# westlake-repl/IDvs.MoRec

Hardware: AMD Instinct MI355X
Metric: user-sequences/sec end-to-end train step, SASRec+BERT-base (higher is better)
Workload: dtype fp16

## Files before the change

### idvs/morec_amd/_lib.py

```python
from __future__ import annotations

import ctypes as C
import os

import torch

_HERE = os.path.dirname(os.path.abspath(__file__))
LIB_PATH = os.environ.get("MOREC_HIP_LIB") or os.path.join(_HERE, "libmorec_hip.so")

F32, BF16, F16 = 0, 1, 2
ACT_NONE, ACT_GELU, ACT_RELU = 0, 1, 2
DACT_MUL = 3


class MorecError(RuntimeError):
    pass


class GemmDesc(C.Structure):
    _fields_ = [("M", C.c_int), ("N", C.c_int), ("K", C.c_int), ("lda", C.c_int), ("ldb", C.c_int), ("ldc", C.c_int),
                ("in_dtype", C.c_int), ("out_dtype", C.c_int), ("act", C.c_int), ("dact", C.c_int),
                ("accumulate", C.c_int), ("split_k", C.c_int), ("alpha", C.c_float), ("aux_deriv", C.c_int)]


# ... 59 lines not shown
    "morec_colsum": (C.c_int, [_P, _P, C.c_int, C.c_int, C.c_int, C.c_int, _P]),
    "morec_layernorm_fwd": (C.c_int, [_P, _P, _P, _P, C.c_int, _P, _P, C.c_float, _P, _P, _P, _P, C.c_int, C.c_int,
                                      C.c_int, C.c_float, C.c_uint64, C.c_float, C.c_uint64, _P, C.c_int, _P]),
    "morec_layernorm_bwd": (C.c_int, [_P, _P, _P, _P, _P, _P, _P, _P, _P, _P, _P, C.c_int, C.c_int, C.c_int, C.c_float,
                                      C.c_uint64, C.c_float, C.c_uint64, _P, _P, C.c_int, _P]),
    "morec_layernorm_fwd_res32": (C.c_int, [_P, _P, _P, _P, C.c_int, _P, _P, C.c_float, _P, _P, _P, _P, _P, C.c_int, C.c_int,
                                            C.c_int, C.c_float, C.c_uint64, C.c_float, C.c_uint64, _P]),
    "morec_layernorm_fwd_res32_pre": (C.c_int, [_P, _P, _P, _P, _P, _P, _P, _P, _P, C.c_float, _P, _P, _P, _P, C.c_int, C.c_int, C.c_int,
                                                C.c_float, C.c_uint64, _P]),
    "morec_layernorm_bwd_res32": (C.c_int, [_P, _P, _P, _P, _P, _P, _P, _P, _P, _P, _P, C.c_int, C.c_int, C.c_int, C.c_float,
                                            C.c_uint64, C.c_float, C.c_uint64, _P]),
    "morec_pos_grad": (C.c_int, [_P, _P, C.c_int, C.c_int, C.c_int, C.c_int, _P]),
    "morec_attn_fwd": (C.c_int, [C.POINTER(AttnDesc), _P, _P, _P, _P]),
    "morec_attn_bwd": (C.c_int, [C.POINTER(AttnDesc), _P, _P, _P, _P, _P]),
    "morec_attn_bwd_dbias": (C.c_int, [C.POINTER(AttnDesc), _P, _P, _P, _P, C.c_int, _P, _P, C.c_size_t, _P]),
    "morec_bert_embed_fwd": (C.c_int, [_P, _P, _P, _P, _P, _P, C.c_float, _P, _P, _P, _P, C.c_int, C.c_int, C.c_int,
                                       C.c_int, C.c_float, C.c_uint64, _P]),
    "morec_bert_embed_bwd": (C.c_int, [_P, _P, _P, _P, _P, C.c_int, C.c_int, C.c_int, C.c_int, C.c_int, _P, _P]),
    "morec_gather_rows": (C.c_int, [_P, _P, _P, C.c_int, C.c_int, C.c_int, _P]),
    "morec_scatter_add_rows": (C.c_int, [_P, _P, _P, C.c_int, C.c_int, C.c_int, C.c_int, _P]),
    "morec_indexed_rows_copy": (C.c_int, [_P, _P, _P, _P, C.c_int, C.c_int, C.c_int, _P]),
    "morec_strided_rows_copy": (C.c_int, [_P, _P, C.c_int, C.c_int, C.c_int, C.c_int, C.c_int, _P]),
    "morec_inbatch_ce_workspace_bytes": (C.c_size_t, [C.POINTER(CeDesc)]),
    "morec_inbatch_ce_fwd": (C.c_int, [C.POINTER(CeDesc), _P, _P, _P, _P, _P, _P, _P, _P, _P, _P, _P, _P]),
    "morec_inbatch_ce_bwd": (C.c_int, [C.POINTER(CeDesc), _P, _P, _P, _P, _P, _P, _P, _P, _P, C.c_float, _P, _P, _P,
                                       _P]),
    "morec_bce_fwd": (C.c_int, [_P, _P, _P, _P, _P, C.c_int, C.c_int, C.c_int, C.c_int, _P]),
    "morec_bce_bwd": (C.c_int, [_P, _P, _P, _P, _P, _P, _P, C.c_int, C.c_int, C.c_int, C.c_int, _P]),
    "morec_adamw": (C.c_int, [_P, _P, _P, _P, _P, C.c_size_t, C.c_float, C.c_float, C.c_float, C.c_float, C.c_float,
                              C.c_int, C.c_float, _P]),
# ... 60 lines not shown
```

### idvs/morec_amd/csrc/attention.hip

```cpp
#include <stdio.h>
#include <stdlib.h>
#include "common.hpp"

namespace {
template <int TB>
struct Tile {
    static constexpr int TP = 8 * TB;
    static constexpr int PP = TP + 4;
};

struct AttnArgs {
    const void* qkv;
    const float* key_keep;
    void* ctx;
    void* dqkv;
    int n_seq, T, n_heads, dh;
    int causal;
    float scale, mask_value;
    DropRng drop;
    const int32_t* cu;
    int total_rows;
};

template <typename T, int DC, int TB>
// ... 610 lines not shown
int check_desc(const morec_attn_desc* d) {
    if (!d) return MOREC_E_ARG;
    if (d->n_seq <= 0 || d->T <= 0 || d->n_heads <= 0 || d->dh <= 0) return MOREC_E_ARG;
    if (d->T > T_MAX) return MOREC_E_UNSUPPORTED;
    if (d->dh % 8) return MOREC_E_ALIGN;
    if (d->p_drop < 0.f || d->p_drop >= 1.f) return MOREC_E_ARG;
    if (d->total_rows < 0 || d->spare_rows_max < 0 || (d->spare_rows_max > 0 && (!d->cu_seqlens || d->total_rows <= 0))) return MOREC_E_ARG;
    return MOREC_OK;
}
}
int attn_spare_blocks(const morec_attn_desc* d) { return (d->cu_seqlens && d->total_rows > 0) ? (d->spare_rows_max + 15) / 16 : 0; }

int morec_attn_mfma_launch(const morec_attn_desc* d, const void* qkv, const float* key_keep, void* ctx_or_dctx,
                           void* dqkv, bool backward, hipStream_t s, float* csum = nullptr);
int colsum_f32_launch(const float* in, float* out, int rows, int N, hipStream_t s);
int morec_attn_f32mfma_launch(const morec_attn_desc* d, const void* qkv, const float* key_keep, void* ctx_or_dctx, void* dqkv, bool backward,
                              hipStream_t s);

static void warn_valu_fallback(const morec_attn_desc* d) {
    if (!is_h16(d->dtype)) return;
    static const bool once = [](const morec_attn_desc* q) {
        if (!tuning().quiet)
            fprintf(stderr, "libmorec_hip: attention with T = %d, head width %d is outside the MFMA path (T <= 64, head width %% 32 == 0): "
                            "running the VALU kernels for this and every later such call\n", q->T, q->dh);
        return true;
    }(d);
    (void)once;
}

extern "C" int morec_attn_fwd(const morec_attn_desc* d, const void* qkv, const float* key_keep, void* ctx,
// ... 40 lines not shown
    if (rc) return rc;
    if (!qkv || !key_keep || !dctx || !dqkv || !dbias || rows <= 0) return MOREC_E_ARG;
    const int H3 = 3 * d->n_heads * d->dh;
    hipStream_t s = reinterpret_cast<hipStream_t>(stream);
    if (ws && ws_bytes >= (size_t)d->n_seq * H3 * sizeof(float)) {
        ws = morec_fold_workspace(ws, (size_t)d->n_seq * H3, s);
        if (!ws) return (int)hipErrorOutOfMemory;
        rc = morec_attn_mfma_launch(d, qkv, key_keep, const_cast<void*>(dctx), dqkv, true, s, ws);
        if (rc == MOREC_OK) return colsum_f32_launch(ws, dbias, d->n_seq, H3, s);
        if (rc != MOREC_E_UNSUPPORTED) return rc;
    }
    rc = morec_attn_bwd(d, qkv, key_keep, dctx, dqkv, stream);
    if (rc) return rc;
    return morec_colsum(dqkv, dbias, rows, H3, H3, d->dtype, stream);
}
```

### idvs/morec_amd/csrc/attention_mfma.hip

```cpp
#include <stdlib.h>
#include "common.hpp"

namespace {
constexpr int DCH = 64;
constexpr int PITCH = DCH * 2 + 32;
constexpr int TILE = 32 * PITCH;
constexpr int PP = 32 * 2 + 32;
typedef __attribute__((ext_vector_type(4))) short s16x4_t;
typedef __attribute__((address_space(3))) s16x4_t* lds_s16x4_ptr;

struct AttnMArgs {
    const bf16* qkv;
    const float* key_keep;
    bf16* ctx;
    bf16* dqkv;
    float* csum;
    int n_seq, T, n_heads, dh, causal;
    float scale, mask_value;
    DropRng drop;
    const int32_t* cu;
    int total_rows;
};


// ... 78 lines not shown
    return __builtin_bit_cast(bf16x8_t, v);
}

__device__ __forceinline__ void load_keep(const AttnMArgs& a, const float* keep_row, float (&keep)[2][4]) {
    const int g = threadIdx.x >> 4;
#pragma unroll
    for (int kb = 0; kb < 2; ++kb)
#pragma unroll
        for (int r = 0; r < 4; ++r) {
            const int j = kb * 16 + 4 * g + r;
            const float v = keep_row[min(j, a.T - 1)];
            keep[kb][r] = (j < a.T) ? v : 0.f;
        }
}

__device__ __forceinline__ void softmax_regs(f32x4_t (&s)[2][2], const AttnMArgs& a, const float (&keep)[2][4]) {
    const int lane = threadIdx.x, c = lane & 15, g = lane >> 4;
#pragma unroll
    for (int qb = 0; qb < 2; ++qb) {
        const int i = qb * 16 + c;
        float m = -INFINITY;
#pragma unroll
        for (int kb = 0; kb < 2; ++kb)
#pragma unroll
            for (int r = 0; r < 4; ++r) {
                const int j = kb * 16 + 4 * g + r;
                const bool kept = (keep[kb][r] != 0.f) && (!a.causal || j <= i);
                const float v = s[qb][kb][r] * a.scale + (kept ? 0.f : a.mask_value);
                s[qb][kb][r] = (j < a.T) ? v : -INFINITY;
                m = fmaxf(m, s[qb][kb][r]);
            }
        m = rows4_max(m);
        float sum = 0.f;
#pragma unroll
// ... 1 lines not shown
#pragma unroll
            for (int r = 0; r < 4; ++r) {
                const float e = (kb * 16 + 4 * g + r < a.T) ? expf(s[qb][kb][r] - m) : 0.f;
                s[qb][kb][r] = e;
                sum += e;
            }
        sum = rows4_sum(sum);
        const float inv = (i < a.T) ? 1.0f / sum : 0.f;
#pragma unroll
        for (int kb = 0; kb < 2; ++kb)
#pragma unroll
            for (int r = 0; r < 4; ++r) s[qb][kb][r] *= inv;
    }
}

__device__ __forceinline__ void drop_mask_regs(const DropRng& d, uint64_t tile, float (&m)[2][2][4]) {
    const int lane = threadIdx.x, c = lane & 15, g = lane >> 4;
#pragma unroll
    for (int qb = 0; qb < 2; ++qb)
#pragma unroll
        for (int kb = 0; kb < 2; ++kb)
        {
            bool kp[4];
            drop_keep_vec<4>(d, (tile * 32 + (uint64_t)(qb * 16 + c)) * 32 + (uint64_t)(kb * 16 + 4 * g), kp);
#pragma unroll
            for (int r = 0; r < 4; ++r) m[qb][kb][r] = kp[r] ? d.inv_keep : 0.f;
        }
}

template <typename T16, int NB>
__device__ __forceinline__ void fwd_pv(const AttnMArgs& a, const char* sV, const bf16x8_t (&pf)[2], size_t row0, int H, int col0) {
    const int lane = threadIdx.x, c = lane & 15, g = lane >> 4;
    const f32x4_t zero = {0.f, 0.f, 0.f, 0.f};
    bf16x8_t vf[NB];
// ... 276 lines not shown
    const bf16x8_t pT[2] = {frag_tr(sP, PP, 0), frag_tr(sP, PP, 16)};
    for (int ch = 0; ch < nch; ++ch) {
        const int d0 = ch * DCH, nc = min(DCH, a.dh - d0);
        if (nch > 1) {
            __syncthreads();
            stage_tile(a.qkv, row0, pitch, head * a.dh + d0, nc, a.T, sQ);
            stage_tile(a.qkv, row0, pitch, H + head * a.dh + d0, nc, a.T, sK);
            stage_tile(dctx, row0, H, head * a.dh + d0, nc, a.T, sO);
            __syncthreads();
        }
        if (nc == 64) bwd_products<T16, 4>(a, sQ, sK, sO, dsf, dsT, pT, row0, pitch, H, head * a.dh + d0, seq);
        else bwd_products<T16, 2>(a, sQ, sK, sO, dsf, dsT, pT, row0, pitch, H, head * a.dh + d0, seq);
    }
}

}

int attn_spare_blocks(const morec_attn_desc* d);
int morec_attn_mfma64_launch(const morec_attn_desc* d, const void* qkv, const float* key_keep, void* ctx_or_dctx, void* dqkv, bool backward,
                             hipStream_t s, float* csum);
int morec_attn_mfma_launch(const morec_attn_desc* d, const void* qkv, const float* key_keep, void* ctx_or_dctx,
                           void* dqkv, bool backward, hipStream_t s, float* csum) {
    if (is_h16(d->dtype) && d->dh % 32 == 0 && d->T > 32 && d->T <= 64) {
        if (tuning().attn_mfma64) return morec_attn_mfma64_launch(d, qkv, key_keep, ctx_or_dctx, dqkv, backward, s, csum);
    }
    if (!is_h16(d->dtype) || d->dh % 32 != 0 || d->T > 32) return MOREC_E_UNSUPPORTED;
    AttnMArgs a{reinterpret_cast<const bf16*>(qkv), key_keep, reinterpret_cast<bf16*>(ctx_or_dctx),
                reinterpret_cast<bf16*>(dqkv), csum, d->n_seq, d->T, d->n_heads, d->dh, d->causal, d->scale, d->mask_value,
                make_drop(d->p_drop, d->seed), d->cu_seqlens, d->total_rows};
    dim3 grid(d->n_seq * d->n_heads + attn_spare_blocks(d)), block(64);
    by_h16(d->dtype, [&](auto* t) {
        using T = MOREC_TAG_T(t);
        if (backward)
            hipLaunchKernelGGL(attn_bwd_mfma_kernel<T>, grid, block, 0, s, a);
        else
            hipLaunchKernelGGL(attn_fwd_mfma_kernel<T>, grid, block, 0, s, a);
    });
    MOREC_CHECK_LAUNCH();
    return MOREC_OK;
}
```

### idvs/morec_amd/csrc/tuning.hip

```cpp
#include <stdlib.h>
#include <string.h>
#include "common.hpp"

namespace {
enum Handling {
    RAW,
    FLAG,
    TMR,
    RESERVE,
    TAIL_BIAS,
    AT_LEAST_1,
    NOT_CHAR_0,
    IS_CHAR_1,
    EPI,
};
struct Row {
    const char* key;
    const char* env;
    int Tuning::*field;
    int def;
    Handling how;
};
const Row ROWS[] = {
    {"gemm8p", "MOREC_GEMM8P", &Tuning::gemm8p, 0, RAW},
    {"gemm2w", "MOREC_GEMM2W", &Tuning::gemm2w, 0, RAW},
    {"gemm_small", "MOREC_GEMM_SMALL", &Tuning::gemm_small, 0, RAW},
    {"gemm_skinny", "MOREC_GEMM_SKINNY", &Tuning::gemm_skinny, 0, RAW},
    {"ce8p", "MOREC_CE8P", &Tuning::ce8p, 0, RAW},
    {"gemm8p_tmr", "MOREC_GEMM8P_TMR", &Tuning::gemm8p_tmr, 1, TMR},
    {"gemm8p_ngroup", "MOREC_GEMM8P_NGROUP", &Tuning::gemm8p_ngroup, -1, RAW},
    {"gemm8p_reserve_cus", "MOREC_GEMM8P_RESERVE_CUS", &Tuning::gemm8p_reserve_cus, 0, RESERVE},
    {"gemm8p_tail_split", "MOREC_GEMM8P_TAIL_SPLIT", &Tuning::gemm8p_tail_split, 0, FLAG},
    {"gemm8p_tail_bias", nullptr, &Tuning::gemm8p_tail_bias, 2, TAIL_BIAS},
    {"gemm8p_debug", "MOREC_GEMM8P_DEBUG", &Tuning::gemm8p_debug, 0, RAW},
    {"gemm8p_stamps_lo", nullptr, &Tuning::gemm8p_stamps_lo, 0, RAW},
    {"gemm8p_stamps_hi", nullptr, &Tuning::gemm8p_stamps_hi, 0, RAW},
    {"deterministic", "MOREC_DETERMINISTIC", &Tuning::deterministic, 0, FLAG},
    {"fold_defer", "MOREC_FOLD_DEFER", &Tuning::fold_defer, 1, FLAG},
    {nullptr, "MOREC_GEMM_TILE", &Tuning::gemm_tile, 0, RAW},
    {nullptr, "MOREC_GEMM_EPI", &Tuning::gemm_epi, 2, EPI},
    {nullptr, "MOREC_GEMM2W_STAGGER", &Tuning::gemm2w_stagger, 0, RAW},
    {nullptr, "MOREC_TN8P_SKIP", &Tuning::tn8p_skip, 1, FLAG},
    {nullptr, "MOREC_ATTN_MFMA64", &Tuning::attn_mfma64, 1, NOT_CHAR_0},
    {nullptr, "MOREC_ATTN_F32_MFMA", &Tuning::attn_f32_mfma, 1, NOT_CHAR_0},
    {nullptr, "MOREC_SWIN_WPW_MIN", &Tuning::swin_wpw_min, 8, AT_LEAST_1},
    {nullptr, "MOREC_SWIN_BWD_WIDE", &Tuning::swin_bwd_wide, 1, RAW},
    {nullptr, "MOREC_QUIET", &Tuning::quiet, 0, IS_CHAR_1},
};

int handled(Handling how, int v) {
    switch (how) {
        case FLAG: return v != 0;
        case TMR: return (v == 0 || v == 1 || v == 224 || v == 192) ? v : 1;
// ... 55 lines not shown
```

### idvs/morec_amd/csrc/tuning.hpp

```cpp
#pragma once

struct Tuning {
    int gemm8p, gemm2w, gemm_small, gemm_skinny, ce8p;
    int gemm8p_tmr;
    int gemm8p_ngroup;
    int gemm8p_reserve_cus;
    int gemm8p_tail_split, gemm8p_tail_bias;
    int gemm8p_debug;
    int gemm8p_stamps_lo, gemm8p_stamps_hi;
    int deterministic;
    int fold_defer;
    int gemm_tile;
    int gemm_epi;
    int gemm2w_stagger;
    int tn8p_skip;
    int attn_mfma64;
    int attn_f32_mfma;
    int swin_wpw_min;
    int swin_bwd_wide;
    int quiet;

    unsigned long long gemm8p_stamps() const {
        return ((unsigned long long)(unsigned)gemm8p_stamps_hi << 32) | (unsigned)gemm8p_stamps_lo;
    }
};

// ... 5 lines not shown
```

### idvs/morec_amd/engine.py

```python
from __future__ import annotations

import math
import os
from dataclasses import dataclass

import torch

from . import ops
from ._lib import ACT_GELU, ACT_RELU, DACT_MUL


@dataclass
class LayerCfg:
    H: int
    heads: int
    T: int
    act: int
    eps: float
    causal: bool
    mask_value: float
    res32: bool = False


_GOLD = 0x9E3779B97F4A7C15
# ... 170 lines not shown
    if cu is None:
        return ops.strided_rows_copy(xc, out, n_seq, xc.shape[1], 1, T)
    return ops.indexed_rows_copy(xc, out, out_idx=cu, R=n_seq)


def layer_forward_cls(cfg: LayerCfg, w: dict, x0: torch.Tensor, key_keep: torch.Tensor, n_seq: int, need_grad: bool,
                      drop: DropCfg = NO_DROP, site0: int = 0, cu=None):
    dh = cfg.H // cfg.heads
    H, T = cfg.H, cfg.T
    x0r = None
    if cfg.res32:
        x0, x0r = x0
    desc = ops.attn_desc(n_seq, T, cfg.heads, dh, cfg.causal, 1.0 / math.sqrt(dh), cfg.mask_value, x0.dtype,
                         drop.p_attn, drop.site(site0), cu, total_rows=x0.shape[0])
    ph, s1, s2 = drop.p_hidden, drop.site(site0 + 1), drop.site(site0 + 2)
    qkv = ops.gemm_nt(x0, w["qkv"].w, bias=w["bqkv"])
    ctx = ops.attn_fwd(desc, qkv, key_keep)
    ctx_c = gather_cls(ctx, n_seq, T, cu)
    if cfg.res32 and isinstance(x0r, ops.PreLN):
        x0_c = x0r.rows(idx=cu[:-1]) if cu is not None else x0r.rows(stride=T, n=n_seq)
    else:
        x0_c = gather_cls(x0r if cfg.res32 else x0, n_seq, T, cu)
    a = ops.gemm_nt(ctx_c, w["o"].w)
    if cfg.res32:
        x1, x1r, z1, mean1, rstd1 = ops.layernorm_fwd_res32(a, w["ln1_g"], w["ln1_b"], cfg.eps, bias=w["bo"], res=x0_c, p_in=ph, seed_in=s1,
                                                            lazy_out=RES32_LAZY)
    else:
        x1, z1, mean1, rstd1 = ops.layernorm_fwd(a, w["ln1_g"], w["ln1_b"], cfg.eps, bias=w["bo"], res=x0_c, z_inplace=True,
                                                 p_in=ph, seed_in=s1)
    u = torch.empty((n_seq, w["f1"].w.shape[0]), device=x0.device, dtype=x0.dtype) if need_grad else None
    g = ops.gemm_nt(x1, w["f1"].w, bias=w["b1"], act=cfg.act, aux_out=u, aux_deriv=need_grad)
    f = ops.gemm_nt(g, w["f2"].w)
    if cfg.res32:
        x2, _, z2, mean2, rstd2 = ops.layernorm_fwd_res32(f, w["ln2_g"], w["ln2_b"], cfg.eps, bias=w["b2"], res=x1r, p_in=ph, seed_in=s2,
                                                          lazy_out=RES32_LAZY)
    else:
        x2, z2, mean2, rstd2 = ops.layernorm_fwd(f, w["ln2_g"], w["ln2_b"], cfg.eps, bias=w["b2"], res=x1, z_inplace=True,
                                                 p_in=ph, seed_in=s2)
    saved = (desc, x0, qkv, ctx_c, z1, mean1, rstd1, x1, u, g, z2, mean2, rstd2, key_keep, ph, s1, s2, n_seq, cu) if need_grad else None
    return x2, saved


def layer_backward_cls(cfg: LayerCfg, w: dict, saved, dx2_c: torch.Tensor, g: dict, need_dx: bool = True):
    desc, x0, qkv, ctx_c, z1, mean1, rstd1, x1, u, gact, z2, mean2, rstd2, key_keep, ph, s1, s2, n_seq, cu = saved
    H, T = cfg.H, cfg.T
    dz2, dzd2 = ops.layernorm_bwd(dx2_c, None, z2, mean2, rstd2, w["ln2_g"], g["ln2_g"], g["ln2_b"], p_in=ph, seed_in=s2,
                                  dbias=g.get("b2"))
    linear_wgrad_(dzd2, gact, g["f2"])
    du = ops.gemm_nt(dzd2, w["f2"].wt, dact=DACT_MUL, dact_in=u, K=dzd2.shape[1], N=u.shape[1], colsum_out=g.get("b1"))
    linear_wgrad_(du, x1, g["f1"])
    dx1 = ops.gemm_nt(du, w["f1"].wt, K=du.shape[1], N=H)
    dz1, dzd1 = ops.layernorm_bwd(dx1, dz2, z1, mean1, rstd1, w["ln1_g"], g["ln1_g"], g["ln1_b"], p_in=ph, seed_in=s1,
                                  dbias=g.get("bo"))
    linear_wgrad_(dzd1, ctx_c, g["o"])
    dctx_c = ops.gemm_nt(dzd1, w["o"].wt, K=dzd1.shape[1], N=H)
    dctx = torch.zeros((x0.shape[0], H), device=dctx_c.device, dtype=dctx_c.dtype)
    scatter_cls(dctx_c, dctx, n_seq, T, cu)
    dqkv = ops.attn_bwd(desc, qkv, key_keep, dctx, dbias=g.get("bqkv"))
    linear_wgrad_(dqkv, x0, g["qkv"])
    if not need_dx:
        return None, None
    dx0 = ops.gemm_nt(dqkv, w["qkv"].wt, K=dqkv.shape[1], N=H)
    if dz1.dtype == dctx.dtype:
        dres = dctx.zero_()
    else:
        dres = torch.zeros((x0.shape[0], H), device=dz1.device, dtype=dz1.dtype)
    scatter_cls(dz1, dres, n_seq, T, cu)
    return dx0, dres


# ... 337 lines not shown
```

### idvs/morec_amd/ops.py

```python
from __future__ import annotations

import ctypes as C
import os

import torch

from . import _lib
from ._lib import ACT_GELU, ACT_NONE, ACT_RELU, BF16, F16, F32, AttnDesc, CeDesc, GemmDesc, SwinAttnDesc, check

FLT_MIN_MASK = -3.4028234663852886e38


DETERMINISTIC = _lib.env_flag("MOREC_DETERMINISTIC")


def set_deterministic(on: bool = True):
    global DETERMINISTIC
    check(_lib.lib().morec_tuning_set(b"deterministic", int(bool(on))), "morec_tuning_set(deterministic)")
    DETERMINISTIC = bool(on)


def code(dt: torch.dtype) -> int:
    if dt == torch.float32:
        return F32
# ... 35 lines not shown
    check(_lib.lib().morec_fold_defer_end(), "morec_fold_defer_end")


def fold_stats() -> dict:
    out = (C.c_ulonglong * 4)()
    check(_lib.lib().morec_fold_stats(out), "morec_fold_stats")
    return {"allocations": out[0], "scratch_bytes": out[1], "jobs": out[2], "launches": out[3]}


def _dev(t):
    if not t.is_cuda:
        raise _lib.MorecError("libmorec_hip needs device tensors (no CPU fallback)")
    if not t.is_contiguous():
        raise _lib.MorecError("tensor must be contiguous")
    return t


def is16(dt: torch.dtype) -> bool:
    return dt in (torch.bfloat16, torch.float16)


def pad8(n: int) -> int:
    return (n + 7) & ~7


FP32_GEMM = "exact"


class fp32_gemm_mode:

# ... 72 lines not shown
        grown = 0
        if ws is not None:
            _WS_RETIRED.append(ws)
            grown = ws.numel() + ws.numel() // 2
        ws = torch.empty(max(need, floor, grown), device=device, dtype=torch.float32)
        cache[device] = ws
    return ws


_GEMM_DESCS = {}


def gemm_nt(a, b, *, bias=None, act=ACT_NONE, out=None, out_dtype=None, aux_out=None, dact=ACT_NONE, dact_in=None,
            accumulate=0, split_k=1, alpha=1.0, M=None, N=None, K=None, lda=None, ldb=None, ldc=None, colsum_out=None,
            aux_deriv=False):
    _dev(a), _dev(b)
    M = a.shape[0] if M is None else M
    K = a.shape[1] if K is None else K
    N = b.shape[0] if N is None else N
    lda = a.stride(0) if lda is None else lda
    ldb = b.stride(0) if ldb is None else ldb
    if out is None:
        out = torch.empty((M, N), device=a.device, dtype=out_dtype or a.dtype)
    ldc = out.stride(0) if ldc is None else ldc
    if FP32_GEMM == "bf16x3" and a.dtype == torch.float32 and b.dtype == torch.float32 and K % 8 == 0:
        whole = a.dim() == 2 and a.is_contiguous() and M == a.shape[0] and K == a.shape[1] and lda == K
        a = split_cached(a) if whole else split_bf16x3(a, 2, M, K, lda)
        b = split_bf16x3(b, 1, N, K, ldb)
        K, lda, ldb = 3 * K, 3 * K, 3 * K
    key = (M, N, K, lda, ldb, ldc, a.dtype, out.dtype, act, dact, accumulate, split_k, alpha, bool(aux_deriv))
    d = _GEMM_DESCS.get(key)
# ... 35 lines not shown
    assert dy.is_contiguous() and x.is_contiguous() and w2t.is_contiguous() and w1.is_contiguous()
    assert x.shape == (M, K) and w1.shape == (N, K) and w2t.shape == (N, K)
    out = torch.empty((M, N), device=dy.device, dtype=dy.dtype)
    ws = None
    if colsum_out is not None:
        ws = _scratch(_DR_WS, dy.device, _lib.lib().morec_mlp_dact_recompute_workspace_bytes(N) // 4, 1024 * 1024)
    check(_lib.lib().morec_mlp_dact_recompute(_p(dy), _p(w2t), _p(x), _p(w1), _p(b1), _p(out), _p(colsum_out), _p(ws), M, N, K,
                                              code(dy.dtype), _stream()), "morec_mlp_dact_recompute")
    return out


_TN_WS = {}


def gemm_tn_(dy, x, out, split_m=1, accumulate=True, slabs=True, stream=None):
    _dev(dy), _dev(x)
    M, N = dy.shape
    K = x.shape[1]
    ws = None
    if slabs and split_m > 1:
        need = _lib.lib().morec_gemm_tn_workspace_bytes(N, K, split_m) // 4
        ws = _scratch(_TN_WS, dy.device, need, 20 * 1024 * 1024)
    check(_lib.lib().morec_gemm_tn(_p(dy), _p(x), _p(out), M, N, K, dy.stride(0), x.stride(0), out.stride(0), code(dy.dtype),
                                   split_m, int(accumulate), _p(ws), _stream() if stream is None else stream), "morec_gemm_tn")
    return out


def transpose(x, out=None, out_dtype=None, ld_out=None):
    _dev(x)
    R, Cc = x.shape
    ld_out = pad8(R) if ld_out is None else ld_out
# ... 167 lines not shown
    return ctx


def attn_bwd(desc, qkv, key_keep, dctx, dbias=None):
    _dev(dctx)
    dqkv = torch.empty_like(qkv)
    if dbias is None:
        check(_lib.lib().morec_attn_bwd(C.byref(desc), _p(qkv), _p(key_keep), _p(dctx), _p(dqkv), _stream()), "morec_attn_bwd")
    else:
        ws = torch.empty((desc.n_seq, qkv.shape[1]), device=qkv.device, dtype=torch.float32)
        check(_lib.lib().morec_attn_bwd_dbias(C.byref(desc), _p(qkv), _p(key_keep), _p(dctx), _p(dqkv), qkv.shape[0], _p(dbias),
                                              _p(ws), ws.numel() * 4, _stream()), "morec_attn_bwd_dbias")
    return dqkv


def bert_embed_fwd(ids32, word, pos, type0, gamma, beta, eps, T, dtype, p_out=0.0, seed_out=0):
    M = ids32.numel()
    H = word.shape[1]
    z = torch.empty((M, H), device=word.device, dtype=dtype)
    y = torch.empty_like(z)
    mean = torch.empty(M, device=word.device, dtype=torch.float32)
    rstd = torch.empty(M, device=word.device, dtype=torch.float32)
    check(_lib.lib().morec_bert_embed_fwd(_p(ids32), _p(word), _p(pos), _p(type0), _p(gamma), _p(beta), eps, _p(z),
                                          _p(y), _p(mean), _p(rstd), M, T, H, code(dtype), p_out, seed_out, _stream()),
          "morec_bert_embed_fwd")
    return y, z, mean, rstd


def bert_embed_bwd_(ids32, dz, dword, dpos, dtype0, pad_id, T, order=None):
    M, H = dz.shape
# ... 287 lines not shown
```

### include/morec_hip.h

```cpp
#ifndef MOREC_HIP_H
#define MOREC_HIP_H

#include <stddef.h>
#include <stdint.h>

#ifdef __cplusplus
extern "C" {
#endif

#define MOREC_F32 0
#define MOREC_BF16 1
#define MOREC_F16 2

#define MOREC_OK 0
#define MOREC_E_ARG (-1)
#define MOREC_E_ALIGN (-2)
#define MOREC_E_UNSUPPORTED (-3)
#define MOREC_E_DTYPE (-4)
#define MOREC_E_COMM (-5)

#define MOREC_ACT_NONE 0
#define MOREC_ACT_GELU 1
#define MOREC_ACT_RELU 2
#define MOREC_DACT_MUL 3
// ... 98 lines not shown
    int causal;
    float scale, mask_value;
    int dtype;
    float p_drop;
    uint64_t seed;
    const int32_t* cu_seqlens;
    int total_rows;
    int spare_rows_max;
} morec_attn_desc;

int morec_attn_fwd(const morec_attn_desc* d, const void* qkv, const float* key_keep, void* ctx, void* stream);
int morec_attn_bwd(const morec_attn_desc* d, const void* qkv, const float* key_keep, const void* dctx, void* dqkv,
                   void* stream);
int morec_attn_bwd_dbias(const morec_attn_desc* d, const void* qkv, const float* key_keep, const void* dctx, void* dqkv,
                         int rows, float* dbias, float* ws, size_t ws_bytes, void* stream);

typedef struct {
    int n_img, H, W;
    int window;
    int shift;
    int heads, dh;
    float scale;
    int dtype;
} morec_swin_attn_desc;
int morec_swin_attn_fwd(const morec_swin_attn_desc* d, const void* qkv, const float* bias_t, void* ctx, void* stream);
int morec_swin_attn_bwd(const morec_swin_attn_desc* d, const void* qkv, const float* bias_t, const void* ctx,
                        const void* dctx, void* dqkv, float* dbias_t, void* stream);
int morec_swin_attn_bwd_dbias(const morec_swin_attn_desc* d, const void* qkv, const float* bias_t, const void* ctx,
                              const void* dctx, void* dqkv, float* dbias_t, float* dbqkv, float* ws, size_t ws_bytes, void* stream);
int morec_swin_bias_expand(const float* table, float* bias_t, int window, int heads, void* stream);
// ... 104 lines not shown
```

Before: 3585.

## Compute only CLS-row queries in last BERT layer attention

In the final encoder layer only the CLS output is consumed, so the QKV projection now computes Q only for CLS rows and K/V for all rows. New single-query attention forward and backward kernels run one wavefront per sequence-head, and the backward pass computes input gradients from the reduced dQ plus the full dK/dV. This removes the Q projection and attention work for non-CLS rows, at the cost of extra gather/scatter ops and new kernels that are gated by a tuning flag and only used for short sequences.

```diff
diff --git a/idvs/morec_amd/_lib.py b/idvs/morec_amd/_lib.py
--- a/idvs/morec_amd/_lib.py
+++ b/idvs/morec_amd/_lib.py
@@ -97,6 +97,9 @@
     "morec_attn_fwd": (C.c_int, [C.POINTER(AttnDesc), _P, _P, _P, _P]),
     "morec_attn_bwd": (C.c_int, [C.POINTER(AttnDesc), _P, _P, _P, _P, _P]),
     "morec_attn_bwd_dbias": (C.c_int, [C.POINTER(AttnDesc), _P, _P, _P, _P, C.c_int, _P, _P, C.c_size_t, _P]),
+    "morec_attn_cls_supported": (C.c_int, [C.POINTER(AttnDesc)]),
+    "morec_attn_cls_fwd": (C.c_int, [C.POINTER(AttnDesc), _P, _P, _P, _P, _P]),
+    "morec_attn_cls_bwd": (C.c_int, [C.POINTER(AttnDesc), _P, _P, _P, _P, _P, _P, _P, _P, C.c_size_t, _P]),
     "morec_bert_embed_fwd": (C.c_int, [_P, _P, _P, _P, _P, _P, C.c_float, _P, _P, _P, _P, C.c_int, C.c_int, C.c_int,
                                        C.c_int, C.c_float, C.c_uint64, _P]),
     "morec_bert_embed_bwd": (C.c_int, [_P, _P, _P, _P, _P, C.c_int, C.c_int, C.c_int, C.c_int, C.c_int, _P, _P]),
diff --git a/idvs/morec_amd/csrc/attention.hip b/idvs/morec_amd/csrc/attention.hip
--- a/idvs/morec_amd/csrc/attention.hip
+++ b/idvs/morec_amd/csrc/attention.hip
@@ -648,6 +648,8 @@
 int morec_attn_mfma_launch(const morec_attn_desc* d, const void* qkv, const float* key_keep, void* ctx_or_dctx,
                            void* dqkv, bool backward, hipStream_t s, float* csum = nullptr);
 int colsum_f32_launch(const float* in, float* out, int rows, int N, hipStream_t s);
+int morec_attn_cls_launch(const morec_attn_desc* d, const void* q_c, const void* kv, const float* key_keep, void* ctx_c_or_dctx_c, void* dkv,
+                          void* dqkv_c, bool backward, hipStream_t s, float* csum);
 int morec_attn_f32mfma_launch(const morec_attn_desc* d, const void* qkv, const float* key_keep, void* ctx_or_dctx, void* dqkv, bool backward,
                               hipStream_t s);
 
@@ -718,3 +720,33 @@
     if (rc) return rc;
     return morec_colsum(dqkv, dbias, rows, H3, H3, d->dtype, stream);
 }
+
+extern "C" int morec_attn_cls_supported(const morec_attn_desc* d) {
+    if (check_desc(d) != MOREC_OK || !tuning().cls_query) return 0;
+    return is_h16(d->dtype) && d->T <= 32 && d->dh % 32 == 0 && d->dh <= 64;
+}
+
+extern "C" int morec_attn_cls_fwd(const morec_attn_desc* d, const void* q_c, const void* kv, const float* key_keep, void* ctx_c, void* stream) {
+    int rc = check_desc(d);
+    if (rc) return rc;
+    if (!q_c || !kv || !key_keep || !ctx_c) return MOREC_E_ARG;
+    if (!aligned16(q_c) || !aligned16(kv) || !aligned16(ctx_c)) return MOREC_E_ALIGN;
+    return morec_attn_cls_launch(d, q_c, kv, key_keep, ctx_c, nullptr, nullptr, false, reinterpret_cast<hipStream_t>(stream), nullptr);
+}
+
+extern "C" int morec_attn_cls_bwd(const morec_attn_desc* d, const void* q_c, const void* kv, const float* key_keep, const void* dctx_c,
+                                  void* dkv, void* dqkv_c, float* dbias, float* ws, size_t ws_bytes, void* stream) {
+    int rc = check_desc(d);
+    if (rc) return rc;
+    if (!q_c || !kv || !key_keep || !dctx_c || !dkv || !dqkv_c) return MOREC_E_ARG;
+    if (!aligned16(q_c) || !aligned16(kv) || !aligned16(dctx_c) || !aligned16(dkv) || !aligned16(dqkv_c)) return MOREC_E_ALIGN;
+    hipStream_t s = reinterpret_cast<hipStream_t>(stream);
+    if (!dbias) return morec_attn_cls_launch(d, q_c, kv, key_keep, const_cast<void*>(dctx_c), dkv, dqkv_c, true, s, nullptr);
+    const int H3 = 3 * d->n_heads * d->dh;
+    if (!ws || ws_bytes < (size_t)d->n_seq * H3 * sizeof(float)) return MOREC_E_ARG;
+    ws = morec_fold_workspace(ws, (size_t)d->n_seq * H3, s);
+    if (!ws) return (int)hipErrorOutOfMemory;
+    rc = morec_attn_cls_launch(d, q_c, kv, key_keep, const_cast<void*>(dctx_c), dkv, dqkv_c, true, s, ws);
+    if (rc) return rc;
+    return colsum_f32_launch(ws, dbias, d->n_seq, H3, s);
+}
diff --git a/idvs/morec_amd/csrc/attention_mfma.hip b/idvs/morec_amd/csrc/attention_mfma.hip
--- a/idvs/morec_amd/csrc/attention_mfma.hip
+++ b/idvs/morec_amd/csrc/attention_mfma.hip
@@ -1,4 +1,5 @@
 #include <stdlib.h>
+#include <type_traits>
 #include "common.hpp"
 
 namespace {
@@ -116,10 +117,11 @@
         }
 }
 
-__device__ __forceinline__ void softmax_regs(f32x4_t (&s)[2][2], const AttnMArgs& a, const float (&keep)[2][4]) {
-    const int lane = threadIdx.x, c = lane & 15, g = lane >> 4;
-#pragma unroll
-    for (int qb = 0; qb < 2; ++qb) {
+template <int NQ>
+__device__ __forceinline__ void softmax_regs(f32x4_t (&s)[NQ][2], const AttnMArgs& a, const float (&keep)[2][4]) {
+    const int lane = threadIdx.x, c = lane & 15, g = lane >> 4;
+#pragma unroll
+    for (int qb = 0; qb < NQ; ++qb) {
         const int i = qb * 16 + c;
         float m = -INFINITY;
 #pragma unroll
@@ -151,10 +153,11 @@
     }
 }
 
-__device__ __forceinline__ void drop_mask_regs(const DropRng& d, uint64_t tile, float (&m)[2][2][4]) {
-    const int lane = threadIdx.x, c = lane & 15, g = lane >> 4;
-#pragma unroll
-    for (int qb = 0; qb < 2; ++qb)
+template <int NQ>
+__device__ __forceinline__ void drop_mask_regs(const DropRng& d, uint64_t tile, float (&m)[NQ][2][4]) {
+    const int lane = threadIdx.x, c = lane & 15, g = lane >> 4;
+#pragma unroll
+    for (int qb = 0; qb < NQ; ++qb)
 #pragma unroll
         for (int kb = 0; kb < 2; ++kb)
         {
@@ -461,6 +464,253 @@
     }
 }
 
+struct AttnCArgs {
+    AttnMArgs m;
+    const bf16* q_c;
+    bf16* dqkv_c;
+};
+
+__device__ __forceinline__ bf16x8_t frag_row_global(const bf16* __restrict__ row, int col) {
+    return __builtin_bit_cast(bf16x8_t, load16(row + col + (threadIdx.x >> 4) * 8));
+}
+
+__device__ __forceinline__ void write_row0_tile_lds(char* __restrict__ tile, uint4 v) {
+    const uint4 z = make_uint4(0, 0, 0, 0);
+    const uint4 t[4] = {threadIdx.x < 8 ? v : z, z, z, z};
+    write_tile_lds(tile, t);
+}
+
+template <typename T16>
+__global__ __launch_bounds__(64) void attn_fwd_cls_kernel(AttnCArgs ca) {
+    AttnMArgs& a = ca.m;
+    a.drop = drop_resolve(a.drop);
+    __shared__ __attribute__((aligned(16))) char sV[TILE];
+    const int lane = threadIdx.x, c = lane & 15, g = lane >> 4;
+    const int seq = blockIdx.x / a.n_heads, head = blockIdx.x % a.n_heads;
+    const int H = a.n_heads * a.dh, pitch = 2 * H;
+    const size_t row0 = a.cu ? (size_t)a.cu[seq] : (size_t)seq * a.T;
+    if (a.cu) a.T = a.cu[seq + 1] - a.cu[seq];
+    if (a.T <= 0) {
+        if (lane * 8 < a.dh) *reinterpret_cast<uint4*>(a.ctx + (size_t)seq * H + head * a.dh + lane * 8) = make_uint4(0, 0, 0, 0);
+        return;
+    }
+    const f32x4_t zero = {0.f, 0.f, 0.f, 0.f};
+    f32x4_t s[1][2] = {{zero, zero}};
+    float keep[2][4];
+    load_keep(a, a.key_keep + row0, keep);
+    uint4 pv[4];
+    load_tile_regs(a.qkv, row0, pitch, H + head * a.dh, a.dh, a.T, pv);
+    bf16x8_t qf[2], kf[2][2];
+    const bf16* qrow = ca.q_c + (size_t)seq * H;
+#pragma unroll
+    for (int ks = 0; ks < 2; ++ks) {
+        const bool ok = ks * 32 < a.dh;
+        const int dcol = head * a.dh + (ok ? ks * 32 : 0);
+        qf[ks] = frag_row_global(qrow, dcol);
+#pragma unroll
+        for (int b = 0; b < 2; ++b) kf[ks][b] = frag_nt_global(a.qkv, row0, pitch, dcol, b, a.T);
+    }
+    __builtin_amdgcn_sched_barrier(0);
+    write_tile_lds(sV, pv);
+#pragma unroll
+    for (int ks = 0; ks < 2; ++ks) {
+        if (ks * 32 < a.dh) {
+#pragma unroll
+            for (int kb = 0; kb < 2; ++kb) s[0][kb] = h16<T16>::mma16(kf[ks][kb], qf[ks], s[0][kb]);
+        }
+    }
+    __syncthreads();
+    softmax_regs<1>(s, a, keep);
+    if (a.drop.thresh) {
+        float m[1][2][4];
+        drop_mask_regs<1>(a.drop, blockIdx.x, m);
+#pragma unroll
+        for (int kb = 0; kb < 2; ++kb)
+#pragma unroll
+            for (int r = 0; r < 4; ++r) s[0][kb][r] *= m[0][kb][r];
+    }
+    const bf16x8_t pf = frag_regs<T16>(s[0]);
+    auto pv_store = [&](auto nb_tag) {
+        constexpr int NB = decltype(nb_tag)::value;
+        f32x4_t o[NB];
+#pragma unroll
+        for (int db = 0; db < NB; ++db) o[db] = h16<T16>::mma16(frag_tr_spread(sV, PITCH, 4 * db, 4 * NB), pf, zero);
+        if (c == 0) store_row_d<T16, NB>(a.ctx, (size_t)seq, H, head * a.dh + 4 * NB * g, o);
+    };
+    if (a.dh == 64) pv_store(std::integral_constant<int, 4>{});
+    else pv_store(std::integral_constant<int, 2>{});
+}
+
+template <typename T16, int NB>
+__device__ __forceinline__ void bwd_products_cls(const AttnCArgs& ca, const char* sQ, const char* sK, const char* sO, const bf16x8_t& dsf0,
+                                                 const bf16x8_t (&dsT)[2], const bf16x8_t (&pT)[2], size_t row0, int H, int col0, int seq) {
+    const AttnMArgs& a = ca.m;
+    const int lane = threadIdx.x, c = lane & 15, g = lane >> 4;
+    const int pitch = 2 * H;
+    const f32x4_t zero = {0.f, 0.f, 0.f, 0.f};
+    f32x4_t ck[NB], cv[NB];
+#pragma unroll
+    for (int db = 0; db < NB; ++db) { ck[db] = zero; cv[db] = zero; }
+    bf16x8_t kt[NB], qt[NB], ot[NB];
+#pragma unroll
+    for (int db = 0; db < NB; ++db) {
+        kt[db] = frag_tr_spread(sK, PITCH, 4 * db, 4 * NB);
+        qt[db] = frag_tr_spread(sQ, PITCH, 4 * db, 4 * NB);
+        ot[db] = frag_tr_spread(sO, PITCH, 4 * db, 4 * NB);
+    }
+    const int dcol = col0 + 4 * NB * g;
+    f32x4_t dq[NB];
+#pragma unroll
+    for (int db = 0; db < NB; ++db) dq[db] = h16<T16>::mma16(kt[db], dsf0, zero);
+    if (c == 0) store_row_d<T16, NB>(ca.dqkv_c, (size_t)seq, 3 * H, dcol, dq);
+#pragma unroll
+    for (int b = 0; b < 2; ++b) {
+        const int r = b * 16 + c;
+        f32x4_t dk[NB], dv[NB];
+#pragma unroll
+        for (int db = 0; db < NB; ++db) {
+            dk[db] = h16<T16>::mma16(qt[db], dsT[b], zero);
+            dv[db] = h16<T16>::mma16(ot[db], pT[b], zero);
+        }
+        if (r < a.T) {
+            store_row_d<T16, NB>(a.dqkv, row0 + r, pitch, dcol, dk);
+            store_row_d<T16, NB>(a.dqkv, row0 + r, pitch, H + dcol, dv);
+            if (r == 0) {
+                store_row_d<T16, NB>(ca.dqkv_c, (size_t)seq, 3 * H, H + dcol, dk);
+                store_row_d<T16, NB>(ca.dqkv_c, (size_t)seq, 3 * H, 2 * H + dcol, dv);
+            }
+            if (a.csum) {
+#pragma unroll
+                for (int db = 0; db < NB; ++db)
+#pragma unroll
+                    for (int e = 0; e < 4; ++e) {
+                        ck[db][e] += dk[db][e];
+                        cv[db][e] += dv[db][e];
+                    }
+            }
+        }
+    }
+    if (a.csum) {
+#pragma unroll
+        for (int db = 0; db < NB; ++db)
+#pragma unroll
+            for (int e = 0; e < 4; ++e) {
+                ck[db][e] = row16_sum(ck[db][e]);
+                cv[db][e] = row16_sum(cv[db][e]);
+            }
+        if (c == 0) {
+            float* w = a.csum + (size_t)seq * 3 * H + dcol;
+#pragma unroll
+            for (int db = 0; db < NB; ++db) {
+                *reinterpret_cast<float4*>(w + 4 * db) = make_float4(dq[db][0], dq[db][1], dq[db][2], dq[db][3]);
+                *reinterpret_cast<float4*>(w + H + 4 * db) = make_float4(ck[db][0], ck[db][1], ck[db][2], ck[db][3]);
+                *reinterpret_cast<float4*>(w + 2 * H + 4 * db) = make_float4(cv[db][0], cv[db][1], cv[db][2], cv[db][3]);
+            }
+        }
+    }
+}
+
+template <typename T16>
+__global__ __launch_bounds__(64) void attn_bwd_cls_kernel(AttnCArgs ca) {
+    AttnMArgs& a = ca.m;
+    if ((int)blockIdx.x >= a.n_seq * a.n_heads) {
+        zero_dead_rows(a.dqkv, a.cu, a.n_seq, a.total_rows, (size_t)2 * a.n_heads * a.dh * 2, (int)blockIdx.x - a.n_seq * a.n_heads);
+        return;
+    }
+    a.drop = drop_resolve(a.drop);
+    __shared__ __attribute__((aligned(16))) char sQ[TILE];
+    __shared__ __attribute__((aligned(16))) char sK[TILE];
+    __shared__ __attribute__((aligned(16))) char sO[TILE];
+    __shared__ __attribute__((aligned(16))) char sP[32 * PP];
+    __shared__ __attribute__((aligned(16))) char sS[32 * PP];
+    const int lane = threadIdx.x, c = lane & 15, g = lane >> 4;
+    const int seq = blockIdx.x / a.n_heads, head = blockIdx.x % a.n_heads;
+    const int H = a.n_heads * a.dh, pitch = 2 * H;
+    const size_t row0 = a.cu ? (size_t)a.cu[seq] : (size_t)seq * a.T;
+    if (a.cu) a.T = a.cu[seq + 1] - a.cu[seq];
+    if (a.T <= 0) {
+        if (a.csum)
+            for (int j = lane; j < 3 * a.dh; j += 64) a.csum[(size_t)seq * 3 * H + (j / a.dh) * H + head * a.dh + j % a.dh] = 0.f;
+        for (int j = lane * 8; j < 3 * a.dh; j += 64 * 8)
+            *reinterpret_cast<uint4*>(ca.dqkv_c + (size_t)seq * 3 * H + (j / a.dh) * H + head * a.dh + j % a.dh) = make_uint4(0, 0, 0, 0);
+        return;
+    }
+    const f32x4_t zero = {0.f, 0.f, 0.f, 0.f};
+    f32x4_t s[1][2] = {{zero, zero}}, dp[1][2] = {{zero, zero}};
+    float keep[2][4];
+    load_keep(a, a.key_keep + row0, keep);
+    const bf16* qrow = ca.q_c + (size_t)seq * H;
+    const bf16* orow = a.ctx + (size_t)seq * H;
+    uint4 pk[4];
+    load_tile_regs(a.qkv, row0, pitch, head * a.dh, a.dh, a.T, pk);
+    const int pcol = head * a.dh + ((lane & 7) * 8 < a.dh ? (lane & 7) * 8 : 0);
+    const uint4 q0 = load16(qrow + pcol), o0 = load16(orow + pcol);
+    bf16x8_t vf[2][2], qf[2], of[2];
+#pragma unroll
+    for (int ks = 0; ks < 2; ++ks) {
+        const bool ok = ks * 32 < a.dh;
+        const int dcol = head * a.dh + (ok ? ks * 32 : 0);
+        qf[ks] = frag_row_global(qrow, dcol);
+        of[ks] = frag_row_global(orow, dcol);
+#pragma unroll
+        for (int b = 0; b < 2; ++b) vf[ks][b] = frag_nt_global(a.qkv, row0, pitch, H + dcol, b, a.T);
+    }
+    __builtin_amdgcn_sched_barrier(0);
+    write_tile_lds(sK, pk);
+    write_row0_tile_lds(sQ, q0);
+    write_row0_tile_lds(sO, o0);
+    __syncthreads();
+#pragma unroll
+    for (int ks = 0; ks < 2; ++ks) {
+        if (ks * 32 < a.dh) {
+            const bf16x8_t kf[2] = {frag_nt(sK, 0, ks), frag_nt(sK, 1, ks)};
+#pragma unroll
+            for (int kb = 0; kb < 2; ++kb) {
+                s[0][kb] = h16<T16>::mma16(kf[kb], qf[ks], s[0][kb]);
+                dp[0][kb] = h16<T16>::mma16(vf[ks][kb], of[ks], dp[0][kb]);
+            }
+        }
+    }
+    softmax_regs<1>(s, a, keep);
+    float msk[1][2][4];
+    if (a.drop.thresh) drop_mask_regs<1>(a.drop, blockIdx.x, msk);
+    {
+        float delta = 0.f;
+#pragma unroll
+        for (int kb = 0; kb < 2; ++kb)
+#pragma unroll
+            for (int r = 0; r < 4; ++r) {
+                if (a.drop.thresh) dp[0][kb][r] *= msk[0][kb][r];
+                delta += s[0][kb][r] * dp[0][kb][r];
+            }
+        delta = rows4_sum(delta);
+        const uint2 z2 = make_uint2(0, 0);
+#pragma unroll
+        for (int kb = 0; kb < 2; ++kb) {
+#pragma unroll
+            for (int r = 0; r < 4; ++r) {
+                dp[0][kb][r] = s[0][kb][r] * (dp[0][kb][r] - delta) * a.scale;
+                if (a.drop.thresh) s[0][kb][r] *= msk[0][kb][r];
+                if (c != 0) {
+                    dp[0][kb][r] = 0.f;
+                    s[0][kb][r] = 0.f;
+                }
+            }
+            const int k0 = kb * 16 + 4 * g;
+            *reinterpret_cast<uint2*>(sP + c * PP + k0 * 2) = make_uint2(h16<T16>::pack2(s[0][kb][0], s[0][kb][1]), h16<T16>::pack2(s[0][kb][2], s[0][kb][3]));
+            *reinterpret_cast<uint2*>(sS + c * PP + k0 * 2) = make_uint2(h16<T16>::pack2(dp[0][kb][0], dp[0][kb][1]), h16<T16>::pack2(dp[0][kb][2], dp[0][kb][3]));
+            *reinterpret_cast<uint2*>(sP + (16 + c) * PP + k0 * 2) = z2;
+            *reinterpret_cast<uint2*>(sS + (16 + c) * PP + k0 * 2) = z2;
+        }
+    }
+    const bf16x8_t dsf0 = frag_regs<T16>(dp[0]);
+    __syncthreads();
+    const bf16x8_t dsT[2] = {frag_tr(sS, PP, 0), frag_tr(sS, PP, 16)};
+    const bf16x8_t pT[2] = {frag_tr(sP, PP, 0), frag_tr(sP, PP, 16)};
+    if (a.dh == 64) bwd_products_cls<T16, 4>(ca, sQ, sK, sO, dsf0, dsT, pT, row0, H, head * a.dh, seq);
+    else bwd_products_cls<T16, 2>(ca, sQ, sK, sO, dsf0, dsT, pT, row0, H, head * a.dh, seq);
+}
+
 }
 
 int attn_spare_blocks(const morec_attn_desc* d);
@@ -486,3 +736,22 @@
     MOREC_CHECK_LAUNCH();
     return MOREC_OK;
 }
+
+int morec_attn_cls_launch(const morec_attn_desc* d, const void* q_c, const void* kv, const float* key_keep, void* ctx_c_or_dctx_c, void* dkv,
+                          void* dqkv_c, bool backward, hipStream_t s, float* csum) {
+    if (!is_h16(d->dtype) || d->dh % 32 != 0 || d->dh > DCH || d->T > 32) return MOREC_E_UNSUPPORTED;
+    AttnCArgs a{{reinterpret_cast<const bf16*>(kv), key_keep, reinterpret_cast<bf16*>(ctx_c_or_dctx_c), reinterpret_cast<bf16*>(dkv), csum,
+                 d->n_seq, d->T, d->n_heads, d->dh, d->causal, d->scale, d->mask_value, make_drop(d->p_drop, d->seed), d->cu_seqlens,
+                 d->total_rows},
+                reinterpret_cast<const bf16*>(q_c), reinterpret_cast<bf16*>(dqkv_c)};
+    dim3 block(64);
+    by_h16(d->dtype, [&](auto* t) {
+        using T = MOREC_TAG_T(t);
+        if (backward)
+            hipLaunchKernelGGL(attn_bwd_cls_kernel<T>, dim3(d->n_seq * d->n_heads + attn_spare_blocks(d)), block, 0, s, a);
+        else
+            hipLaunchKernelGGL(attn_fwd_cls_kernel<T>, dim3(d->n_seq * d->n_heads), block, 0, s, a);
+    });
+    MOREC_CHECK_LAUNCH();
+    return MOREC_OK;
+}
diff --git a/idvs/morec_amd/csrc/tuning.hip b/idvs/morec_amd/csrc/tuning.hip
--- a/idvs/morec_amd/csrc/tuning.hip
+++ b/idvs/morec_amd/csrc/tuning.hip
@@ -37,6 +37,7 @@
     {"gemm8p_stamps_hi", nullptr, &Tuning::gemm8p_stamps_hi, 0, RAW},
     {"deterministic", "MOREC_DETERMINISTIC", &Tuning::deterministic, 0, FLAG},
     {"fold_defer", "MOREC_FOLD_DEFER", &Tuning::fold_defer, 1, FLAG},
+    {"cls_query", "MOREC_CLS_QUERY", &Tuning::cls_query, 1, FLAG},
     {nullptr, "MOREC_GEMM_TILE", &Tuning::gemm_tile, 0, RAW},
     {nullptr, "MOREC_GEMM_EPI", &Tuning::gemm_epi, 2, EPI},
     {nullptr, "MOREC_GEMM2W_STAGGER", &Tuning::gemm2w_stagger, 0, RAW},
diff --git a/idvs/morec_amd/csrc/tuning.hpp b/idvs/morec_amd/csrc/tuning.hpp
--- a/idvs/morec_amd/csrc/tuning.hpp
+++ b/idvs/morec_amd/csrc/tuning.hpp
@@ -10,6 +10,7 @@
     int gemm8p_stamps_lo, gemm8p_stamps_hi;
     int deterministic;
     int fold_defer;
+    int cls_query;
     int gemm_tile;
     int gemm_epi;
     int gemm2w_stagger;
diff --git a/idvs/morec_amd/engine.py b/idvs/morec_amd/engine.py
--- a/idvs/morec_amd/engine.py
+++ b/idvs/morec_amd/engine.py
@@ -208,13 +208,21 @@
     desc = ops.attn_desc(n_seq, T, cfg.heads, dh, cfg.causal, 1.0 / math.sqrt(dh), cfg.mask_value, x0.dtype,
                          drop.p_attn, drop.site(site0), cu, total_rows=x0.shape[0])
     ph, s1, s2 = drop.p_hidden, drop.site(site0 + 1), drop.site(site0 + 2)
-    qkv = ops.gemm_nt(x0, w["qkv"].w, bias=w["bqkv"])
-    ctx = ops.attn_fwd(desc, qkv, key_keep)
-    ctx_c = gather_cls(ctx, n_seq, T, cu)
+    cls_query = ops.attn_cls_supported(desc)
+    if not cls_query:
+        qkv = ops.gemm_nt(x0, w["qkv"].w, bias=w["bqkv"])
+        ctx = ops.attn_fwd(desc, qkv, key_keep)
+        ctx_c = gather_cls(ctx, n_seq, T, cu)
     if cfg.res32 and isinstance(x0r, ops.PreLN):
         x0_c = x0r.rows(idx=cu[:-1]) if cu is not None else x0r.rows(stride=T, n=n_seq)
     else:
         x0_c = gather_cls(x0r if cfg.res32 else x0, n_seq, T, cu)
+    if cls_query:
+        x0_q = gather_cls(x0, n_seq, T, cu) if cfg.res32 else x0_c
+        bq, bkv = (None, None) if w["bqkv"] is None else (w["bqkv"][:H], w["bqkv"][H:])
+        qkv = ops.gemm_nt(x0, w["qkv"].w[H:], bias=bkv)
+        q_c = ops.gemm_nt(x0_q, w["qkv"].w[:H], bias=bq)
+        ctx_c = ops.attn_cls_fwd(desc, q_c, qkv, key_keep)
     a = ops.gemm_nt(ctx_c, w["o"].w)
     if cfg.res32:
         x1, x1r, z1, mean1, rstd1 = ops.layernorm_fwd_res32(a, w["ln1_g"], w["ln1_b"], cfg.eps, bias=w["bo"], res=x0_c, p_in=ph, seed_in=s1,
@@ -231,7 +239,8 @@
     else:
         x2, z2, mean2, rstd2 = ops.layernorm_fwd(f, w["ln2_g"], w["ln2_b"], cfg.eps, bias=w["b2"], res=x1, z_inplace=True,
                                                  p_in=ph, seed_in=s2)
-    saved = (desc, x0, qkv, ctx_c, z1, mean1, rstd1, x1, u, g, z2, mean2, rstd2, key_keep, ph, s1, s2, n_seq, cu) if need_grad else None
+    saved = (desc, x0, (qkv, q_c, x0_q) if cls_query else qkv, ctx_c, z1, mean1, rstd1, x1, u, g, z2, mean2, rstd2, key_keep, ph, s1, s2, n_seq,
+             cu) if need_grad else None
     return x2, saved
 
 
@@ -248,6 +257,19 @@
                                   dbias=g.get("bo"))
     linear_wgrad_(dzd1, ctx_c, g["o"])
     dctx_c = ops.gemm_nt(dzd1, w["o"].wt, K=dzd1.shape[1], N=H)
+    if isinstance(qkv, tuple):
+        kv, q_c, x0_q = qkv
+        dkv, dqkv_c = ops.attn_cls_bwd(desc, q_c, kv, key_keep, dctx_c, dbias=g.get("bqkv"))
+        linear_wgrad_(dkv, x0, g["qkv"][H:])
+        linear_wgrad_(dqkv_c[:, :H], x0_q, g["qkv"][:H])
+        if not need_dx:
+            return None, None
+        wt = w["qkv"].wt
+        dx0 = ops.gemm_nt(dkv, wt[:, H:], K=2 * H, N=H)
+        scatter_cls(ops.gemm_nt(dqkv_c, wt, K=3 * H, N=H), dx0, n_seq, T, cu)
+        dres = torch.zeros((x0.shape[0], H), device=dz1.device, dtype=dz1.dtype)
+        scatter_cls(dz1, dres, n_seq, T, cu)
+        return dx0, dres
     dctx = torch.zeros((x0.shape[0], H), device=dctx_c.device, dtype=dctx_c.dtype)
     scatter_cls(dctx_c, dctx, n_seq, T, cu)
     dqkv = ops.attn_bwd(desc, qkv, key_keep, dctx, dbias=g.get("bqkv"))
diff --git a/idvs/morec_amd/ops.py b/idvs/morec_amd/ops.py
--- a/idvs/morec_amd/ops.py
+++ b/idvs/morec_amd/ops.py
@@ -73,6 +73,12 @@
     if not t.is_contiguous():
         raise _lib.MorecError("tensor must be contiguous")
     return t
+
+
+def _dev_rows(t):
+    if t.dim() == 2 and t.is_cuda and t.stride(1) == 1 and t.stride(0) >= t.shape[1]:
+        return t
+    return _dev(t)
 
 
 def is16(dt: torch.dtype) -> bool:
@@ -175,7 +181,7 @@
 def gemm_nt(a, b, *, bias=None, act=ACT_NONE, out=None, out_dtype=None, aux_out=None, dact=ACT_NONE, dact_in=None,
             accumulate=0, split_k=1, alpha=1.0, M=None, N=None, K=None, lda=None, ldb=None, ldc=None, colsum_out=None,
             aux_deriv=False):
-    _dev(a), _dev(b)
+    _dev_rows(a), _dev_rows(b)
     M = a.shape[0] if M is None else M
     K = a.shape[1] if K is None else K
     N = b.shape[0] if N is None else N
@@ -241,7 +247,7 @@
 
 
 def gemm_tn_(dy, x, out, split_m=1, accumulate=True, slabs=True, stream=None):
-    _dev(dy), _dev(x)
+    _dev_rows(dy), _dev_rows(x)
     M, N = dy.shape
     K = x.shape[1]
     ws = None
@@ -439,6 +445,27 @@
     return dqkv
 
 
+def attn_cls_supported(desc) -> bool:
+    return bool(_lib.lib().morec_attn_cls_supported(C.byref(desc)))
+
+
+def attn_cls_fwd(desc, q_c, kv, key_keep):
+    _dev(q_c), _dev(kv), _dev(key_keep)
+    ctx_c = torch.empty_like(q_c)
+    check(_lib.lib().morec_attn_cls_fwd(C.byref(desc), _p(q_c), _p(kv), _p(key_keep), _p(ctx_c), _stream()), "morec_attn_cls_fwd")
+    return ctx_c
+
+
+def attn_cls_bwd(desc, q_c, kv, key_keep, dctx_c, dbias=None):
+    _dev(dctx_c)
+    dkv = torch.empty_like(kv)
+    dqkv_c = torch.empty((q_c.shape[0], 3 * q_c.shape[1]), device=kv.device, dtype=kv.dtype)
+    ws = None if dbias is None else torch.empty((desc.n_seq, 3 * q_c.shape[1]), device=kv.device, dtype=torch.float32)
+    check(_lib.lib().morec_attn_cls_bwd(C.byref(desc), _p(q_c), _p(kv), _p(key_keep), _p(dctx_c), _p(dkv), _p(dqkv_c), _p(dbias), _p(ws),
+                                        0 if ws is None else ws.numel() * 4, _stream()), "morec_attn_cls_bwd")
+    return dkv, dqkv_c
+
+
 def bert_embed_fwd(ids32, word, pos, type0, gamma, beta, eps, T, dtype, p_out=0.0, seed_out=0):
     M = ids32.numel()
     H = word.shape[1]
diff --git a/include/morec_hip.h b/include/morec_hip.h
--- a/include/morec_hip.h
+++ b/include/morec_hip.h
@@ -136,6 +136,10 @@
                    void* stream);
 int morec_attn_bwd_dbias(const morec_attn_desc* d, const void* qkv, const float* key_keep, const void* dctx, void* dqkv,
                          int rows, float* dbias, float* ws, size_t ws_bytes, void* stream);
+int morec_attn_cls_supported(const morec_attn_desc* d);
+int morec_attn_cls_fwd(const morec_attn_desc* d, const void* q_c, const void* kv, const float* key_keep, void* ctx_c, void* stream);
+int morec_attn_cls_bwd(const morec_attn_desc* d, const void* q_c, const void* kv, const float* key_keep, const void* dctx_c, void* dkv,
+                       void* dqkv_c, float* dbias, float* ws, size_t ws_bytes, void* stream);
 
 typedef struct {
     int n_img, H, W;
```

Measured after the change: 3603 (median of 6 runs). About the same (+0.5%).
